# fanzyflani/pwnfps

Measured on AMD Instinct MI355X. Metric: Mpixels/s at 3840x2160 (level.txt scene, trace + blur), frames resident on the device; mean steps/ray alongside; d2h_inclusive = the rate with every frame delivered to the host (SURVEY 8d), higher is better.
Workload: dtype f32; 1 GPU; pwnfps level.txt scene (14 game.lua spheres, spawn pose, sec_current=0), 3840x2160, POSTPROC_BLUR=1, one frame per step; level=pwnfps_level, width=3840, height=2160, blur_passes=1, parallelism=rows/1, 3 frames in flight on two compute streams, frames_repeated_with_whole_strips=0

## Files before the change

include/pwnhip.h:

```cpp
#ifndef PWNHIP_H
#define PWNHIP_H
#include <stddef.h>
#include <stdint.h>

#ifdef __cplusplus
extern "C" {
#endif

#define PWN_OK            0
#define PWN_EINVAL       -1
#define PWN_ENODEV       -2
#define PWN_ENOMEM       -3
#define PWN_EIO          -4
#define PWN_EHIP         -5
#define PWN_ENOLEVEL     -6
#define PWN_ETOOBIG      -7
#define PWN_EBUSY        -8
#define PWN_ENOTSUP      -9
#define PWN_ETIMEDOUT    -10

typedef struct pwn_ctx pwn_ctx;

typedef struct pwn_portal { int32_t x1, z1, x2, z2, rot12, c1, c2; } pwn_portal;

// ... 50 lines not shown
	uint64_t frames, frames_redone, recuts;
	char note[160];
} pwn_group_info;
int pwn_init_multi(pwn_ctx **out, const int *devices, int ndev, int width, int height);
int pwn_group_info_get(pwn_ctx *ctx, pwn_group_info *out);
int pwn_set_option(pwn_ctx *ctx, int option, int value);
int pwn_unit_order_state(pwn_ctx *ctx, unsigned long long out[4]);
int pwn_unit_order_probe(pwn_ctx *ctx, const uint16_t *cost, uint32_t units, uint32_t *perm_out);
int pwn_launch_order_waits(pwn_ctx *ctx, unsigned long long *out);
int pwn_trace_room_state(pwn_ctx *ctx, int out[4]);
const char *pwn_strerror(int code);
const char *pwn_last_error(pwn_ctx *ctx);

int pwn_level_load(pwn_ctx *ctx, const char *path);
int pwn_level_load_mem(pwn_ctx *ctx, const char *text, int len);
int pwn_upload_level(pwn_ctx *ctx, const uint8_t data[4096], const pwn_portal pmap[26]);
int pwn_get_level(pwn_ctx *ctx, uint8_t data[4096], pwn_portal pmap[26], int32_t spawn[2]);

int pwn_upload_spheres(pwn_ctx *ctx, const pwn_sphere *spheres, int n);
int pwn_get_bins(pwn_ctx *ctx, uint16_t counts[4096], int32_t *idx, int cap);
#define PWN_TABLES_MAX (16u << 20)
#define PWN_LIST_MAX 4096
int pwn_sphere_tables_plan(const pwn_sphere *spheres, int n, unsigned long long out[6]);
int pwn_sphere_tables_state(pwn_ctx *ctx, unsigned long long out[6]);

#define PWN_OBJ_MAX 10000
int pwn_obj_new(pwn_ctx *ctx);
int pwn_obj_set_sphere(pwn_ctx *ctx, int obj, double r, double refl, double x, double y, double z,
	double cb, double cg, double cr);
int pwn_obj_free(pwn_ctx *ctx, int obj);
int pwn_level_get(pwn_ctx *ctx, int cx, int cz);
int pwn_prepare_render(pwn_ctx *ctx);
int pwn_get_objects(pwn_ctx *ctx, pwn_sphere *out, int cap);

int pwn_trace_screen_centred(pwn_ctx *ctx, const float cam[16], float sec_current,
	uint32_t *sbuf, float *zbuf);
int pwn_host_register(pwn_ctx *ctx, void *base, size_t bytes);
int pwn_host_unregister(pwn_ctx *ctx, void *base);
int pwn_call_strips_state(pwn_ctx *ctx, unsigned long long out[6]);

#define PWN_VIEWS_MAX 1024
int pwn_trace_views(pwn_ctx *ctx, int n, const float *cams, const float *secs, uint32_t *sbuf, float *zbuf);
#define PWN_VIEWS_HAS_W 1
int pwn_trace_views_device(pwn_ctx *ctx, int n, const void *d_cams, const void *d_secs, int flags,
	void *d_work, void *d_sbuf, void *d_zbuf, void *stream);

// ... 140 lines not shown
```

pwnfps_amd/__init__.py:

```python
from .render import (Renderer, PwnError, SPHERE_DTYPE, PORTAL_DTYPE, HIT_DTYPE,
                     mat4_iden, mat4_roty, mat4_rotx, spawn_camera, pixel_rays, unit_order_xy, sphere_tables_plan,
                     viewports_plan)
```

pwnfps_amd/_lib.py:

```python
import ctypes as C
import os

_HERE = os.path.dirname(os.path.abspath(__file__))
LIB_PATH = os.environ.get("PWNHIP_LIB") or os.path.join(_HERE, "libpwnhip.so")

PWN_OK, PWN_EINVAL, PWN_ENODEV, PWN_ENOMEM, PWN_EIO, PWN_EHIP, PWN_ENOLEVEL, PWN_ETOOBIG = 0, -1, -2, -3, -4, -5, -6, -7
PWN_EBUSY, PWN_ENOTSUP, PWN_ETIMEDOUT = -8, -9, -10
PWN_OPT_BLUR_PASSES, PWN_OPT_COUNTERS, PWN_OPT_SCHEDULER, PWN_OPT_REFILL_LIMIT, PWN_OPT_FRAME_TIMING, PWN_OPT_WAVE_LOG = 1, 2, 3, 4, 5, 6
PWN_OPT_FRAME_OVERLAP = 7
PWN_OPT_TRACE_ROOM = 8
PWN_OPT_UNIT_ORDER = 9
PWN_OPT_TILED_CHOREO = 10
PWN_OPT_TILED_STREAMS = 11
PWN_OPT_TILED_COMMS = 12
PWN_OPT_CALL_STRIPS = 13
PWN_TILED_CHOREO_INSTREAM, PWN_TILED_CHOREO_SPLIT = 0, 1
PWN_SCHED_UNITS, PWN_SCHED_REFILL = 0, 1
PWN_MAX_SLOTS = 4
PWN_FRAME_SBUF, PWN_FRAME_ZBUF, PWN_FRAME_SURFACE = 1, 2, 4
PWN_OBJ_MAX = 10000
PWN_TABLES_MAX = 16 << 20
PWN_VIEWS_MAX = 1024
PWN_RAYS_HAS_W = 1
PWN_VIEWS_HAS_W = 1
# ... 59 lines not shown
PWN_TILED_ID_BYTES = 128
PWN_TRANSPORT_RCCL, PWN_TRANSPORT_SHM, PWN_TRANSPORT_LOCAL = 0, 1, 2
PWN_TILED_HOST = 1
PWN_TILED_SLOTS = 6
PWN_TILED_MAX_WORLD = 64

_vp, _i, _f, _d = C.c_void_p, C.c_int, C.c_float, C.c_double
ABI = [
    ("pwn_init", _i, [C.POINTER(_vp), _i, _i, _i]),
    ("pwn_init_multi", _i, [C.POINTER(_vp), _vp, _i, _i, _i]),
    ("pwn_group_info_get", _i, [_vp, C.POINTER(GroupInfo)]),
    ("pwn_destroy", None, [_vp]),
    ("pwn_set_option", _i, [_vp, _i, _i]),
    ("pwn_trace_room_state", _i, [_vp, _vp]),
    ("pwn_strerror", C.c_char_p, [_i]),
    ("pwn_last_error", C.c_char_p, [_vp]),
    ("pwn_level_load", _i, [_vp, C.c_char_p]),
    ("pwn_level_load_mem", _i, [_vp, C.c_char_p, _i]),
    ("pwn_upload_level", _i, [_vp, _vp, _vp]),
    ("pwn_get_level", _i, [_vp, _vp, _vp, _vp]),
    ("pwn_upload_spheres", _i, [_vp, _vp, _i]),
    ("pwn_get_bins", _i, [_vp, _vp, _vp, _i]),
    ("pwn_sphere_tables_plan", _i, [_vp, _i, _vp]),
    ("pwn_sphere_tables_state", _i, [_vp, _vp]),
    ("pwn_obj_new", _i, [_vp]),
    ("pwn_obj_set_sphere", _i, [_vp, _i, _d, _d, _d, _d, _d, _d, _d, _d]),
    ("pwn_obj_free", _i, [_vp, _i]),
    ("pwn_level_get", _i, [_vp, _i, _i]),
    ("pwn_prepare_render", _i, [_vp]),
    ("pwn_get_objects", _i, [_vp, _vp, _i]),
    ("pwn_trace_screen_centred", _i, [_vp, _vp, _f, _vp, _vp]),
    ("pwn_host_register", _i, [_vp, _vp, C.c_size_t]),
    ("pwn_host_unregister", _i, [_vp, _vp]),
    ("pwn_call_strips_state", _i, [_vp, _vp]),
    ("pwn_trace_views", _i, [_vp, _i, _vp, _vp, _vp, _vp]),
    ("pwn_trace_views_device", _i, [_vp, _i, _vp, _vp, _i, _vp, _vp, _vp, _vp]),
    ("pwn_viewports_plan", _i, [_i, _i, _i, _i, _vp, _vp]),
    ("pwn_trace_viewports", _i, [_vp, _i, _vp, _vp, _vp, _vp, _vp]),
    ("pwn_pixel_rays", _i, [_i, _i, _vp, _i, _vp, _vp, _vp]),
    ("pwn_trace_rays", _i, [_vp, _i, _vp, _vp, _f, _vp, _vp]),
    ("pwn_trace_rays_device", _i, [_vp, _i, _vp, _vp, _f, _i, _vp, _vp, _vp]),
    ("pwn_trace_hits", _i, [_vp, _i, _vp, _vp]),
    ("pwn_trace_hits_device", _i, [_vp, _i, _vp, _i, _vp, _vp]),
    ("pwn_get_object_ids", _i, [_vp, _vp, _i]),
    ("pwn_frames_config", _i, [_vp, _i, _i, _i, _i]),
    ("pwn_submit_frame", _i, [_vp, _vp, _f, _i]),
# ... 51 lines not shown
```

pwnfps_amd/csrc/level_host.c:

```c
#include <stdint.h>
#include <stdlib.h>
#include <string.h>
#include "level_host.h"

enum { DIR_XP = 0, DIR_ZP, DIR_XN, DIR_ZN };

static int is_open(int c)
{
	switch(c)
	{
		case ';': case '$': case '"': case '#': case '&':
		case '>': case '<': case '^': case ',':
			return 1;
	}
	return 0;
}

static int flat_cell(const uint8_t *cells, int x, int z)
{
	int i = z * 64 + x;
	return (i >= 0 && i < 4096) ? cells[i] : '.';
}

static const int dir_dx[4] = { 1, 0, -1, 0 };
static const int dir_dz[4] = { 0, 1, 0, -1 };
// ... 156 lines not shown
			int x2 = trunc_to_int(s[i].x + s[i].r), z2 = trunc_to_int(s[i].z + s[i].r);
			if(x1 < 0) x1 = 0;
			if(z1 < 0) z1 = 0;
			if(x2 > 63) x2 = 63;
			if(z2 > 63) z2 = 63;
			for(int z = z1; z <= z2; z++)
			for(int x = x1; x <= x2; x++)
			{
				int c = z * 64 + x;
				if(pass == 0) off[c + 1]++;
				else idx[off[c] + fill[c]++] = i;
			}
		}
		if(pass == 0)
		{
			for(int c = 0; c < 4096; c++) off[c + 1] += off[c];
			if(idx == NULL) { free(fill); return off[4096]; }
			if(off[4096] > idx_cap) { free(fill); return -1; }
		}
	}
	free(fill);
	return off[4096];
}
```

pwnfps_amd/csrc/level_host.h:

```cpp
#ifndef PWN_LEVEL_HOST_H
#define PWN_LEVEL_HOST_H
#include <stdint.h>
#include "pwnhip.h"
#include "cell_bake.h"
#ifdef __cplusplus
extern "C" {
#endif
void pwn_level_clear(uint8_t *cells, pwn_portal *pmap, int32_t *spawn);
int pwn_parse_level(const char *text, int len, uint8_t *cells, pwn_portal *pmap, int32_t *spawn);
int pwn_check_portals(const uint8_t *cells, const pwn_portal *pmap);
int pwn_bake_cells(const uint8_t *cells, const pwn_portal *pmap, uint16_t *bits, uint32_t *recs);
int pwn_bin_spheres(const pwn_sphere *s, int n, int32_t *off, int32_t *idx, int idx_cap);
#ifdef __cplusplus
}
#endif
#endif
```

pwnfps_amd/csrc/pwn_api.cpp:

```cpp
#include <hip/hip_runtime.h>
#include <stdint.h>
#include <stdio.h>
#include <stdlib.h>
#include <string.h>
#include <time.h>
#include <new>
#include <algorithm>
#include <vector>
#include <xmmintrin.h>

#include "pwnhip.h"
#include "pwn_internal.h"
#include "level_host.h"
#include "approx_tables.inc"

extern "C" const char *pwn_strerror(int code)
{
	switch(code)
	{
		case PWN_OK: return "ok";
		case PWN_EINVAL: return "invalid argument";
		case PWN_ENODEV: return "no usable HIP device";
		case PWN_ENOMEM: return "out of memory";
		case PWN_EIO: return "level file could not be read";
// ... 23 lines not shown

#define GRP_HEAD(c) ((c) != NULL && (c)->grp != NULL && (c)->grp_head)
#define GRP_M0(c) pwn_group_member((c), 0)
#define GRP_REFUSE(c, what) do { if(GRP_HEAD(c)) { snprintf((c)->err, sizeof((c)->err), "%s is not available on a group's handle", what); return PWN_ENOTSUP; } } while(0)

extern "C" int pwn_init(pwn_ctx **out, int device, int width, int height)
{
	if(out == NULL || width <= 0 || height <= 0 || width > 32768 || height > 32768) return PWN_EINVAL;
	*out = NULL;
	int ndev = 0;
	if(hipGetDeviceCount(&ndev) != hipSuccess || ndev <= 0 || device < 0 || device >= ndev) return PWN_ENODEV;
	pwn_ctx *c = new(std::nothrow) pwn_ctx();
	if(c == NULL) return PWN_ENOMEM;
	c->device = device; c->w = width; c->h = height;
	c->blur_passes = 1; c->counters_on = 0; c->scheduler = PWN_SCHED_DEFAULT; c->refill_limit = PWN_REFILL_LIMIT_DEFAULT; c->have_level = false; c->cell_base_ok = false;
	if(const char *e = getenv("PWN_SCHEDULER")) c->scheduler = (strcmp(e, "refill") == 0 || strcmp(e, "1") == 0) ? PWN_SCHED_REFILL : PWN_SCHED_UNITS;
	if(const char *e = getenv("PWN_REFILL_LIMIT")) { int v = atoi(e); if(v >= 1 && v <= 64000) c->refill_limit = v; }
	c->dbg_force_hasw = getenv("PWN_DBG_FORCE_HASW") != NULL;
	c->dbg_blocks_per_cu = 0;
	c->dbg_blur_th = 0;
	if(const char *e = getenv("PWN_DBG_BLUR_TH")) c->dbg_blur_th = atoi(e);
	c->dbg_sphere_lists = 0; c->off_recsph = 0;
	c->dbg_sphere_lists = pwn_i_forced_lists();
	c->lists_form = PWN_LF_INDEXED; c->big_which = c->big_sph = 0; c->big_high = 0;
	for(int i = 0; i < PWN_NBLOB; i++) { c->d_big[i] = NULL; c->d_big_cap[i] = 0; }
	for(int i = 0; i < PWN_NSTAGE; i++) { c->h_big[i] = NULL; c->h_big_cap[i] = 0; }
	c->dbg_blur_tw = 0; c->dbg_blur_batch = -1;
	if(const char *e = getenv("PWN_DBG_BLUR_TW")) c->dbg_blur_tw = atoi(e);
	if(const char *e = getenv("PWN_DBG_BLUR_BATCH")) if(*e) c->dbg_blur_batch = atoi(e);
	if(const char *e = getenv("PWN_DBG_BLOCKS_PER_CU")) { int v = atoi(e); if(v > 0) c->dbg_blocks_per_cu = v; }
	c->blob_cur = 0; c->blob_dirty = true; c->off_sph = 0; c->stage_next = 0; c->up_stream = NULL;
	for(int i = 0; i < PWN_NBLOB; i++)
	{
		c->d_blob[i] = NULL; c->blob_has_static[i] = false;
		c->ev_tables[i] = NULL; c->tables_in_use[i] = false; c->tables_wait[i] = NULL;
		c->ev_upload[i] = NULL; c->upload_pending[i] = false;
	}
	for(int i = 0; i < PWN_NSTAGE; i++) { c->h_stage[i] = NULL; c->ev_stage[i] = NULL; c->stage_used[i] = false; }
	c->d_pre = c->d_out = NULL; c->d_z = NULL; c->d_skip = NULL; c->d_counters = NULL; c->d_tickets = NULL; c->ticket_set = 0; c->launch_rot = 2; c->launch_waits = 0;
	c->grid_reserve = 0;
	c->d_vpre = c->d_vout = NULL; c->d_vz = NULL; c->views_cap = 0; c->h_vrec = c->d_vrec = NULL; c->vrec_cap = 0; c->d_vrec_dev = NULL;
	c->d_ppre = c->d_pout = NULL; c->d_pz = NULL; c->h_prec = c->d_prec = NULL;
	c->h_rays = c->d_rays = NULL; c->rays_cap = 0;
	c->h_hits = c->d_hits = NULL; c->hits_cap = 0;
	memset(&c->room, 0, sizeof(c->room)); c->room.mode = -1;
	if(const char *e = getenv("PWN_TRACE_ROOM")) if(*e) c->room.mode = atoi(e) < 0 ? -1 : atoi(e);
// ... 372 lines not shown
			ci[(i >> 6) * PWN_GRID_PITCH + (i & 63)] |= PWN_C_SPH | (ord << 16);
			start[ord++] = (uint32_t)k0;
			for(int32_t k = k0; k < k1; k++)
			{
				const pwn_sphere &q = c->spheres[(size_t)c->bin_idx[k]];
				float r2 = q.r * q.r;
				if(r2 < 1.17549435e-38f) r2 = 0.0f;
				rec[4 * (size_t)k + 0] = q.x; rec[4 * (size_t)k + 1] = q.y; rec[4 * (size_t)k + 2] = q.z;
				uint32_t wbits;
				memcpy(&wbits, &r2, 4);
				if(k == k1 - 1) wbits |= 0x80000000u;
				memcpy(&rec[4 * (size_t)k + 3], &wbits, 4);
				which[k] = (uint32_t)c->bin_idx[k];
			}
		}
	}
	memcpy(b + PWN_T_RCP, c->tabs, 4096);
	memcpy(b + PWN_T_RSQ, c->tabs + 2048, 4096);
	pwn_fill_faces((float *)(b + PWN_T_FACES));
	memcpy(b + PWN_T_EPREC, c->ep_recs, sizeof(c->ep_recs));
	c->off_sph = glb ? 0u : (inl ? pwn_t_sph_offset_inl(nrec) : pwn_t_sph_offset(nbin));
	c->off_recsph = inl ? pwn_t_recsph_offset(nrec) : 0u;
	c->lists_form = plan.form;
	{
		float *sp = glb ? (float *)(c->big.data() + c->big_sph) : (float *)(b + c->off_sph);
		for(uint32_t i = 0; i < nsph; i++, sp += 8)
		{
			const pwn_sphere &q = c->spheres[i];
			float r2 = q.r * q.r;
			if(r2 < 1.17549435e-38f) r2 = 0.0f;
			sp[0] = q.x; sp[1] = q.y; sp[2] = q.z; sp[3] = r2;
			sp[4] = q.refl; sp[5] = q.cb; sp[6] = q.cg; sp[7] = q.cr;
		}
	}

	const int nb = (c->blob_cur + 1) % PWN_NBLOB;
	const uint32_t from = c->blob_has_static[nb] ? PWN_T_CELLINFO : 0u;
	const unsigned st = c->stage_next++ % PWN_NSTAGE;
	if(c->stage_used[st]) HIPCHK(c, hipEventSynchronize(c->ev_stage[st]));
	memcpy(c->h_stage[st], b + from, total - from);
	if(glb)
	{
		const int rc = big_reserve(c, nb, st, c->big.size());
		if(rc != PWN_OK) return rc;
		memcpy(c->h_big[st], c->big.data(), c->big.size());
	}
// ... 249 lines not shown
		if(n > cap) return PWN_EINVAL;
		for(int i = 0; i < n; i++) idx[i] = c->bin_idx[i];
	}
	return n;
}

static void plan_out(const pwn_tables_plan &p, unsigned long long out[6])
{
	out[0] = (unsigned long long)p.form;
	out[1] = (unsigned long long)p.blob_bytes + pwn_trace_lds_extra();
	out[2] = p.big_bytes;
	out[3] = p.nrec; out[4] = p.ncell; out[5] = p.longest;
}

extern "C" int pwn_sphere_tables_plan(const pwn_sphere *s, int n, unsigned long long out[6])
{
	if(out == NULL || n < 0 || n > PWN_OBJ_MAX || s == NULL) return PWN_EINVAL;
	std::vector<int32_t> off(4097, 0);
	if(pwn_bin_spheres(s, n, off.data(), NULL, 0) < 0) return PWN_ENOMEM;
	pwn_tables_plan p;
	const int rc = pwn_i_tables_plan(off.data(), (uint32_t)n, PWN_SCHED_DEFAULT, pwn_i_forced_lists(), &p);
	plan_out(p, out);
	return rc;
}

extern "C" int pwn_sphere_tables_state(pwn_ctx *c, unsigned long long out[6])
{
	if(GRP_HEAD(c)) { const int rc = pwn_group_sync(c); return rc != PWN_OK ? rc : pwn_sphere_tables_state(GRP_M0(c), out); }
	if(c == NULL || out == NULL) return PWN_EINVAL;
	pwn_tables_plan p;
	const int rc = pwn_i_tables_plan(c->bin_off.data(), (uint32_t)c->spheres.size(), c->scheduler, c->dbg_sphere_lists, &p);
	plan_out(p, out);
	return rc;
}



static void unit_div_magic(uint32_t d, uint32_t *magic, int *shift)
{
	*magic = 0u; *shift = -1;
	if(d < 2u) return;
	int s = 0;
	while((2u << s) < d) s++;
	const unsigned long long two = 1ull << (32 + s);
	const unsigned long long M = (two + d - 1u) / d;
	*magic = (uint32_t)M; *shift = s;
// ... 113 lines not shown
	{
		P.vps = vps->d_recs; P.nvp = vps->n; P.tiles_total = (int)vps->units;
		P.vp_step0 = 0u;
		if(vps->n > 1) { P.vp_step0 = 1u; while(2u * P.vp_step0 <= (uint32_t)vps->n - 1u) P.vp_step0 *= 2u; }
	}
	if(rays != NULL)
	{
		P.rays = rays->d_rays; P.ray_seeds = rays->d_seeds; P.nrays = rays->n; P.ray_w = rays->has_w ? 1 : 0;
		P.hits = rays->d_hits;
		P.tiles_total = (int)((rays->n + 63u) / 64u);
	}
	P.blob_bytes = (uint32_t)c->blob.size();
	P.off_sph = c->off_sph;
	P.off_recsph = c->off_recsph;
	P.sbuf = L->d_sbuf; P.zbuf = L->d_zbuf;
	const int cur = c->blob_cur;
	P.blob = (const uint32_t *)c->d_blob[cur];
	const bool glb = c->lists_form == PWN_LF_GLOBAL;
	if(glb)
	{
		P.g_rec = (const float *)c->d_big[cur];
		P.g_which = (const uint32_t *)(c->d_big[cur] + c->big_which);
		P.g_sph = (const float *)(c->d_big[cur] + c->big_sph);
	}
	if(c->upload_pending[cur])
	{
		if(hipEventQuery(c->ev_upload[cur]) == hipSuccess) c->upload_pending[cur] = false;
		else HIPCHK(c, hipStreamWaitEvent(stream, c->ev_upload[cur], 0));
	}
	P.counters = c->d_counters;
	P.clear_word = L->clear_word;
	P.cost_word = L->cost_word;
	P.wave_log = NULL;
	const unsigned rot = (unsigned)c->launch_rot, nsets = 2u * rot;
	P.tickets = c->d_tickets + (c->ticket_set % nsets) * PWN_QUEUES * PWN_QUEUE_STRIDE;
	P.tickets_next = c->d_tickets + ((c->ticket_set + rot) % nsets) * PWN_QUEUES * PWN_QUEUE_STRIDE;
	if(views != NULL) P.has_w = views->has_w;
	else if(rays != NULL) P.has_w = rays->has_w;
	else if(vps != NULL) P.has_w = vps->has_w;
	else P.has_w = !(L->cam[3] == 0.0f && L->cam[7] == 0.0f && L->cam[11] == 0.0f && L->cam[15] == 1.0f);
	if(c->dbg_force_hasw) P.has_w = 1;
	if(c->counters_on) HIPCHK(c, hipMemsetAsync(c->d_counters, 0, PWN_NCOUNTERS * sizeof(unsigned long long), stream));
	const bool refill = c->scheduler == PWN_SCHED_REFILL && !batch && !glb;
	const size_t lds_bytes = ((P.blob_bytes + 15u) & ~15u) + (refill ? pwn_trace_refill_lds_extra(P.has_w != 0) : pwn_trace_lds_extra());
	P.scheduler = c->scheduler;
	P.refill_limit = c->refill_limit;
// ... 1165 lines not shown
```

pwnfps_amd/csrc/pwn_internal.h:

```cpp
#pragma once
#include <hip/hip_runtime.h>
#include <stdint.h>
#include <stdio.h>
#include <vector>
#include <atomic>

#include "pwnhip.h"
#include "tables.h"

struct pwn_views_launch
{
	const pwn_view_rec *d_recs;
	int n;
	bool has_w;
	unsigned long long plane;
};

struct pwn_vps_launch
{
	const pwn_viewport_rec *d_recs, *h_recs;
	int n;
	bool has_w;
	uint32_t units;
};
// ... 125 lines not shown
	uint8_t cells[4096];
	uint32_t cell_base[65 * 65];
	bool cell_base_ok;
	uint32_t ep_recs[PWN_EP_MAX];
	pwn_portal pmap[26];
	int32_t spawn[2];
	std::vector<pwn_sphere> spheres;
	std::vector<int32_t> bin_off, bin_idx;
	std::vector<pwn_sphere> objs;
	std::vector<uint8_t> obj_typ;

	std::vector<uint8_t> blob;
	uint8_t *d_blob[PWN_NBLOB]; int blob_cur;
	bool blob_has_static[PWN_NBLOB];
	hipEvent_t ev_tables[PWN_NBLOB]; bool tables_in_use[PWN_NBLOB];
	hipEvent_t tables_wait[PWN_NBLOB];
	hipEvent_t ev_upload[PWN_NBLOB]; bool upload_pending[PWN_NBLOB];
	uint8_t *h_stage[PWN_NSTAGE]; hipEvent_t ev_stage[PWN_NSTAGE]; bool stage_used[PWN_NSTAGE]; unsigned stage_next;
	hipStream_t up_stream;
	uint16_t tabs[4096];
	uint32_t off_sph;
	uint32_t off_recsph; int dbg_sphere_lists;
	int lists_form;
	std::vector<uint8_t> big; uint64_t big_which, big_sph;
	uint8_t *d_big[PWN_NBLOB]; size_t d_big_cap[PWN_NBLOB];
	uint8_t *h_big[PWN_NSTAGE]; size_t h_big_cap[PWN_NSTAGE];
	size_t big_high;
	bool blob_dirty;
	size_t occ_lds[12]; int occ_blocks[12];

	uint32_t *d_pre, *d_out;
	float *d_z;
	uint2 *d_skip;
	unsigned long long *d_counters;
	unsigned long long *d_wave_log; int wave_log_on; size_t wave_log_cap;
	struct unit_order_state
	{
		hipStream_t key; bool used; unsigned long long stamp;
		uint16_t *d_cost; uint32_t *d_perm; size_t cost_cap, perm_cap;
		uint32_t units, qcap; int y0, y1;
		bool cost_fresh;
		uint32_t perm_units; int perm_y0, perm_y1; bool perm_valid;
	} order[4];
	unsigned long long order_stamp;
	int tiled_choreo;
	int tiled_streams;
// ... 101 lines not shown
```

pwnfps_amd/csrc/tables.h:

```cpp
#pragma once
#include <stdint.h>
#include "cell_bake.h"

#define PWN_GRID_PITCH 65u
#define PWN_T_RCP      0u
#define PWN_T_RSQ      4096u
#define PWN_T_FACES    8192u
#define PWN_T_EXP2     8448u
#define PWN_T_CELLINFO 8704u
#define PWN_T_EPREC    25616u
#define PWN_T_BINIDX   25824u

#define PWN_RCP_BASE   0x7e800000u
#define PWN_RSQ_BASE   0x5f000000u

#define PWN_C_ROOM   0x0100u
#define PWN_C_ROOM2  0x0200u
#define PWN_C_FOG    0x0400u
#define PWN_C_DQ     0x0800u
#define PWN_C_RAMP   0x1000u
#define PWN_C_RAMPX  0x2000u
#define PWN_C_RAMPM  0x4000u
#define PWN_C_PORTAL 0x8000u
#define PWN_C_SPH    0x80000000u
#define PWN_LIST_END 0xffffu
// ... 82 lines not shown
	int refill_limit;
	uint32_t *tickets, *tickets_next;
	uint32_t *cost_word;
	uint16_t *unit_cost;
	const uint32_t *perm;
	uint32_t perm_cap;
	uint32_t *clear_word;
	uint32_t off_recsph;
	const struct pwn_view_rec *views;
	int nviews;
	uint32_t views_magic; int views_shift;
	unsigned long long plane;
	const float *rays;
	const uint32_t *ray_seeds;
	uint32_t nrays;
	int ray_w;
	void *hits;
	const float *g_rec;
	const uint32_t *g_which;
	const float *g_sph;
	const struct pwn_viewport_rec *vps;
	int nvp;
	uint32_t vp_step0;
};
#define PWN_HIT_REC_BYTES 48u

struct pwn_blur_params
{
	int w, h, y0, y1;
	int groups;
	const uint32_t *pre;
	const float *zbuf;
	uint32_t *out;
	const uint2 *skip;
	int avail_y0, avail_y1;
	uint32_t *miss;
	int tile_h, tile_w, batch;
	uint32_t *cost_acc, *cost_out;
	uint32_t cost_mul, cost_div;
	int views;
	unsigned long long plane;
	const struct pwn_viewport_rec *vps;
	int nvp, vp_tiles;
};

enum { PWN_KM_FRAME = 0, PWN_KM_VIEWS = 1, PWN_KM_RAYS = 2, PWN_KM_HITS = 3, PWN_KM_VIEWPORTS = 4 };
// ... 27 lines not shown
```

pwnfps_amd/csrc/trace_common.h:

```cpp
#pragma once
#include <hip/hip_runtime.h>
#include <mutex>
#include "dev_math.h"
#include "tables.h"

#define EPS 0.0000000000001f
#define REFLECT_BLUR_F 0.03f
#define REFLECT_MAX 2
enum { FXP = 0, FZP, FXN, FZN, FYP, FYN };

#ifndef PWN_BLOCK
#define PWN_BLOCK 256
#endif
#define TILE_W 16
#define TILE_H 4

#ifndef PWN_MIN_WAVES
#define PWN_MIN_WAVES 3
#endif

#define PWN_LDS __attribute__((address_space(3)))
template<class T> __device__ __forceinline__ const PWN_LDS T *lds_at(uint32_t byte) { return (const PWN_LDS T *)(uintptr_t)byte; }
typedef float pwn_f4 __attribute__((ext_vector_type(4)));
struct Lds
{
	const PWN_LDS uint32_t *cellinfo;
	const PWN_LDS uint16_t *rcp, *rsq;
	const PWN_LDS unsigned char *eprec;
	const PWN_LDS uint16_t *binidx;
	const PWN_LDS uint16_t *recsph;
	const PWN_LDS float *sph;
	const PWN_LDS uint64_t *exp2;
	const PWN_LDS pwn_f4 *faces;
	const pwn_f4 *g_rec;
	const uint32_t *g_which;
	const pwn_f4 *g_sph;
};
__device__ __forceinline__ Lds lds_tables(uint32_t off_sph, uint32_t off_recsph = 0u)
{
	Lds L;
	L.cellinfo = lds_at<uint32_t>(PWN_T_CELLINFO);
	L.rcp = lds_at<uint16_t>(PWN_T_RCP);
	L.rsq = lds_at<uint16_t>(PWN_T_RSQ);
	L.eprec = lds_at<unsigned char>(PWN_T_EPREC - PWN_PST_REC0 * 4u);
// ... 69 lines not shown
	return r;
}
template<bool W> __device__ __forceinline__ Vec<W> vsub(const Vec<W> &a, const Vec<W> &b)
{
	Vec<W> r; r.x = a.x - b.x; r.y = a.y - b.y; r.z = a.z - b.z;
	if constexpr(W) r.w = a.w - b.w; else r.w = 0.0f;
	return r;
}
template<bool W> __device__ __forceinline__ Vec<W> vnormalise(const PWN_LDS uint16_t *rsq, const Vec<W> &a)
{
	return vscale<W>(tab_rsqrt(rsq, dot3<W>(a, a)), a);
}

__device__ __forceinline__ float dpp_row_shr1(float v)
{
	return __int_as_float(__builtin_amdgcn_update_dpp(0, __float_as_int(v), 0x111 , 0xf, 0xf, true));
}

enum { EV_NONE = 0, EV_WALL, EV_SPHERE, EV_EXHAUSTED };
enum { BASE_CEIL = 0, BASE_FLOOR, BASE_WALL, BASE_MAGENTA, BASE_ROOM_Y };

enum { RG_SEG = 0, RG_SETUP_SLOW, RG_EXHAUSTED, RG_WALL, RG_SPHERE, RG_FLOOR, RG_SPHREFL, RG_JITTER, RG_COMP1, RG_COMP1_FOG,
	RG_COMP2, RG_COMP2_FOG, RG_HELP, RG_UNIT, RG_SPHTEST, RG_SPHUPD, RG_ELSE,
	RG_UNIT_HALF, RG_HC_R2, RG_HC_OUT, RG_PORTAL_WALL, RG_PORTAL_GO, RG_PORTAL_ODD, RG_PORTAL_ROT2, RG_N };
struct Counters { uint32_t rays, steps, portals, tests, exhausted, wsteps, wp[8], apasses, apass_lanes, rg[RG_N]; };
#define WAVE_PATH(k) do { if(COUNT && (__ffsll((long long)__ballot(1)) - 1) == (int)(threadIdx.x & 63)) cnt.wp[k]++; } while(0)
#define RG(k) do { if(COUNT && (__ffsll((long long)__ballot(1)) - 1) == (int)(threadIdx.x & 63)) cnt.rg[k]++; } while(0)


__device__ __forceinline__ uint32_t pixel_seed(int x, int y, int w)
{
	uint32_t seed = (uint32_t)x + (uint32_t)y * (uint32_t)y * ((uint32_t)w + 1u);
	seed *= seed * seed;
	seed *= seed * seed;
	return seed << 1;
}

__device__ __forceinline__ void blob_to_lds(unsigned char *lds, const void *blob, uint32_t blob_bytes)
{
	const uint4 *src = (const uint4 *)blob;
	uint4 *dst = (uint4 *)lds;
	int n16 = (int)(blob_bytes >> 4);
	for(int i = threadIdx.x; i < n16; i += PWN_BLOCK) dst[i] = src[i];
}

__device__ __forceinline__ uint32_t next_open_queue(uint32_t q, unsigned long long open)
{
// ... 75 lines not shown
```

pwnfps_amd/csrc/trace_walk.inc:

```
#define AUX_HIT() (cdist > aux_dist)
if(COUNT)
{
	cnt.steps++;
	if((__ffsll((long long)__ballot(1)) - 1) == (int)(threadIdx.x & 63)) cnt.wsteps++;
}

if constexpr(HITREC) hit_cxz = cxz;

#ifdef PWN_PLAIN_STATS
if(COUNT)
{
	const bool sp1 = ((int)cw < 0) || !(cw & PWN_C_ROOM);
	const bool sp2 = sp1 || (cw & (PWN_C_ROOM2 | PWN_C_DQ)) != 0u;
	const bool low = (__ffsll((long long)__ballot(1)) - 1) == (int)(threadIdx.x & 63);
	if(__ballot(sp1) == 0ull && low) cnt.apasses++;
	if(__ballot(sp2) == 0ull && low) cnt.apass_lanes++;
}
#endif

if((int)cw < 0)
{
	WAVE_PATH(0);
	if constexpr(LISTS == PWN_LF_GLOBAL)
	{
		uint32_t ri = ((const PWN_LDS uint32_t *)L.binidx)[(cw >> 16) & 0x7fffu];
		pwn_f4 nx = L.g_rec[(size_t)ri];
		for(;;)
		{
			RG(RG_SPHTEST);
			const pwn_f4 s0 = nx;
			const uint32_t wb = __float_as_uint(s0.w);
			nx = L.g_rec[(size_t)ri + 1u];
#define PWN_ST_RAD2 __uint_as_float(wb & 0x7fffffffu)
#define PWN_ST_WHICH ri
#include "trace_sphere.inc"
#undef PWN_ST_RAD2
#undef PWN_ST_WHICH
			if((int)wb < 0) break;
			ri++;
		}
	}
	else if constexpr(LISTS == PWN_LF_INLINE)
	{
		const PWN_LDS pwn_f4 *rp = (const PWN_LDS pwn_f4 *)L.binidx + ((cw >> 16) & 0x7fffu);
		pwn_f4 nx = *rp;
		for(;;)
// ... 228 lines not shown
```

pwnfps_amd/render.py:

```python
import ctypes as C

import numpy as np

from . import _lib
from ._lib import lib

HIT_DTYPE = np.dtype([("kind", "<i4"), ("face", "<i4"), ("object", "<i4"), ("portals", "<i4"),
                      ("dist", "<f4"), ("x", "<f4"), ("y", "<f4"), ("z", "<f4"),
                      ("dx", "<f4"), ("dy", "<f4"), ("dz", "<f4"), ("cell_x", "<i2"), ("cell_z", "<i2")])
SPHERE_DTYPE = np.dtype([("r", "<f4"), ("refl", "<f4"), ("x", "<f4"), ("y", "<f4"),
                         ("z", "<f4"), ("cb", "<f4"), ("cg", "<f4"), ("cr", "<f4")])
PORTAL_DTYPE = np.dtype([(n, "<i4") for n in ("x1", "z1", "x2", "z2", "rot12", "c1", "c2")])


class PwnError(RuntimeError):
    def __init__(self, code, where, detail=""):
        self.code = code
        msg = "%s: %s (%d)" % (where, lib.pwn_strerror(code).decode(), code)
        if detail:
            msg += ": " + detail
        super().__init__(msg)


class Renderer:
# ... 514 lines not shown
        words = np.ascontiguousarray(words).view(np.uint32).ravel()
        per = {_lib.PROBE_DIV: 2, _lib.PROBE_FTOINT: 4}.get(op, 1)
        n = words.size // per
        out = np.zeros(n, np.uint32)
        self._chk(lib.pwn_probe(self._ctx, int(op), words.ctypes.data, out.ctypes.data, n), "pwn_probe")
        return out


def _tables_dict(out):
    return {"form": int(out[0]), "lds_bytes": int(out[1]), "device_bytes": int(out[2]), "pairs": int(out[3]),
            "cells": int(out[4]), "longest": int(out[5])}


def sphere_tables_plan(spheres):
    spheres = np.ascontiguousarray(spheres, SPHERE_DTYPE)
    out = (C.c_uint64 * 6)()
    buf = spheres if len(spheres) else np.zeros(1, SPHERE_DTYPE)
    rc = lib.pwn_sphere_tables_plan(buf.ctypes.data, len(spheres), out)
    if rc < 0:
        raise PwnError(rc, "pwn_sphere_tables_plan")
    return _tables_dict(out)


def _rect_records(rects, who):
    rects = np.asarray(rects)
    if rects.ndim != 2 or rects.shape[1] != 4 or rects.shape[0] < 1:
        raise ValueError("%s: rects must have shape (n,4) with n >= 1, not %s" % (who, rects.shape))
    if rects.shape[0] > _lib.PWN_VIEWS_MAX:
        raise ValueError("%s: %d rectangles, at most %d" % (who, rects.shape[0], _lib.PWN_VIEWS_MAX))
    return np.ascontiguousarray(rects, np.int32)


def viewports_plan(W, H, rects, blur):
    rects = _rect_records(rects, "viewports_plan")
    out = (C.c_uint64 * 4)()
    rc = lib.pwn_viewports_plan(int(W), int(H), int(blur), rects.shape[0], rects.ctypes.data, out)
    if rc not in (_lib.PWN_OK, _lib.PWN_EINVAL):
        raise PwnError(rc, "pwn_viewports_plan")
    return {"ok": rc == _lib.PWN_OK, "units": int(out[0]), "pixels": int(out[1]), "largest": int(out[2]), "offender": int(out[3])}


def _ray_records(rays, who):
    if isinstance(rays, (tuple, list)) and len(rays) == 2:
        o, d = np.asarray(rays[0]), np.asarray(rays[1])
        if o.ndim != 2 or d.ndim != 2 or o.shape[0] != d.shape[0] or o.shape[1] not in (3, 4) or d.shape[1] not in (3, 4):
            raise ValueError("%s: origins and directions must be (n,3) or (n,4) with the same n, not %s and %s" % (who, o.shape, d.shape))
# ... 94 lines not shown
```

Measured before the change: 26610 Mpixels/s.

## Cull dense sphere cells with wave-uniform bounding-sphere test

On the host, builds up to four bounding spheres around the most populated sphere-list cells and passes them through the kernel arguments. In the trace walk, when a whole wavefront shares a cell list with such a bound, it runs one conservative ray-vs-bound test. If no lane can hit the bound, it skips the per-sphere tests for that cell. This adds a kernarg read, a ballot and a branch per sphere cell, and relies on the bound staying conservative for correctness.

```diff
diff --git a/include/pwnhip.h b/include/pwnhip.h
--- a/include/pwnhip.h
+++ b/include/pwnhip.h
@@ -96,6 +96,8 @@
 #define PWN_TABLES_MAX (16u << 20)
 #define PWN_LIST_MAX 4096
 int pwn_sphere_tables_plan(const pwn_sphere *spheres, int n, unsigned long long out[6]);
+#define PWN_BOUNDS_MAX 4
+int pwn_sphere_bounds_plan(const pwn_sphere *spheres, int n, double out[PWN_BOUNDS_MAX][8]);
 int pwn_sphere_tables_state(pwn_ctx *ctx, unsigned long long out[6]);
 
 #define PWN_OBJ_MAX 10000
diff --git a/pwnfps_amd/__init__.py b/pwnfps_amd/__init__.py
--- a/pwnfps_amd/__init__.py
+++ b/pwnfps_amd/__init__.py
@@ -1,3 +1,3 @@
 from .render import (Renderer, PwnError, SPHERE_DTYPE, PORTAL_DTYPE, HIT_DTYPE,
-                     mat4_iden, mat4_roty, mat4_rotx, spawn_camera, pixel_rays, unit_order_xy, sphere_tables_plan,
+                     mat4_iden, mat4_roty, mat4_rotx, spawn_camera, pixel_rays, unit_order_xy, sphere_tables_plan, sphere_bounds_plan,
                      viewports_plan)
diff --git a/pwnfps_amd/_lib.py b/pwnfps_amd/_lib.py
--- a/pwnfps_amd/_lib.py
+++ b/pwnfps_amd/_lib.py
@@ -105,6 +105,7 @@
     ("pwn_upload_spheres", _i, [_vp, _vp, _i]),
     ("pwn_get_bins", _i, [_vp, _vp, _vp, _i]),
     ("pwn_sphere_tables_plan", _i, [_vp, _i, _vp]),
+    ("pwn_sphere_bounds_plan", _i, [_vp, _i, _vp]),
     ("pwn_sphere_tables_state", _i, [_vp, _vp]),
     ("pwn_obj_new", _i, [_vp]),
     ("pwn_obj_set_sphere", _i, [_vp, _i, _d, _d, _d, _d, _d, _d, _d, _d]),
diff --git a/pwnfps_amd/csrc/level_host.c b/pwnfps_amd/csrc/level_host.c
--- a/pwnfps_amd/csrc/level_host.c
+++ b/pwnfps_amd/csrc/level_host.c
@@ -1,6 +1,7 @@
 #include <stdint.h>
 #include <stdlib.h>
 #include <string.h>
+#include <math.h>
 #include "level_host.h"
 
 enum { DIR_XP = 0, DIR_ZP, DIR_XN, DIR_ZN };
@@ -203,3 +204,61 @@
 	free(fill);
 	return off[4096];
 }
+
+int pwn_sphere_bounds_build(const pwn_sphere *s, const int32_t *off, const int32_t *idx, int form, pwn_sphere_bound *out)
+{
+	int pick[PWN_BOUNDS_MAX], npick = 0;
+	for(int k = 0; k < PWN_BOUNDS_MAX; k++)
+	{
+		int best = -1, best_n = PWN_BOUND_MIN_RECORDS - 1;
+		for(int c = 0; c < 4096; c++)
+		{
+			const int n = off[c + 1] - off[c];
+			if(n <= best_n) continue;
+			int taken = 0;
+			for(int j = 0; j < npick; j++) taken |= pick[j] == c;
+			if(!taken) { best = c; best_n = n; }
+		}
+		if(best < 0) break;
+		pick[npick++] = best;
+	}
+	int nout = 0;
+	for(int k = 0; k < npick; k++)
+	{
+		const int cell = pick[k], k0 = off[cell], k1 = off[cell + 1], n = k1 - k0;
+		uint32_t id = 0;
+		for(int c = 0; c < cell; c++)
+		{
+			const int m = off[c + 1] - off[c];
+			if(m > 0) id += form == 0 ? (uint32_t)m + 1u : (form == 1 ? (uint32_t)m : 1u);
+		}
+		int ok = 1;
+		double mx = 0.0, my = 0.0, mz = 0.0;
+		for(int i = k0; i < k1; i++)
+		{
+			const pwn_sphere *q = &s[idx[i]];
+			const double v[4] = { q->x, q->y, q->z, q->r };
+			for(int j = 0; j < 4; j++) if(!(fabs(v[j]) <= PWN_SB_COORD_LIMIT)) ok = 0;
+			mx += q->x; my += q->y; mz += q->z;
+		}
+		if(!ok) continue;
+		const float cx = (float)(mx / n), cy = (float)(my / n), cz = (float)(mz / n);
+		double reff = 0.0;
+		for(int i = k0; i < k1; i++)
+		{
+			const pwn_sphere *q = &s[idx[i]];
+			const double dx = (double)q->x - cx, dy = (double)q->y - cy, dz = (double)q->z - cz;
+			const double rho = sqrt(dx * dx + dy * dy + dz * dz) * (1.0 + 1e-12), r = fabs((double)q->r);
+			if(!(rho + r <= PWN_SB_R_LIMIT)) ok = 0;
+			const double a = PWN_SB_D_MAX + rho;
+			const double r0 = rho + sqrt(r * r + PWN_SB_EPS_PROOF * a * a + PWN_SB_ETA);
+			if(r0 > reff) reff = r0;
+		}
+		if(!ok) continue;
+		const float rf = nextafterf((float)(reff * (1.0 + 1.0 / 1048576.0)), INFINITY);
+		const float rr = nextafterf((float)((double)rf * (double)rf), INFINITY);
+		pwn_sphere_bound *b = &out[nout++];
+		b->id = id; b->count = (uint32_t)n; b->cx = cx; b->cy = cy; b->cz = cz; b->rr = rr; b->neg_r = -rf; b->cell = (uint32_t)cell;
+	}
+	return nout;
+}
diff --git a/pwnfps_amd/csrc/level_host.h b/pwnfps_amd/csrc/level_host.h
--- a/pwnfps_amd/csrc/level_host.h
+++ b/pwnfps_amd/csrc/level_host.h
@@ -3,6 +3,7 @@
 #include <stdint.h>
 #include "pwnhip.h"
 #include "cell_bake.h"
+#include "sphere_bound.h"
 #ifdef __cplusplus
 extern "C" {
 #endif
@@ -11,6 +12,7 @@
 int pwn_check_portals(const uint8_t *cells, const pwn_portal *pmap);
 int pwn_bake_cells(const uint8_t *cells, const pwn_portal *pmap, uint16_t *bits, uint32_t *recs);
 int pwn_bin_spheres(const pwn_sphere *s, int n, int32_t *off, int32_t *idx, int idx_cap);
+int pwn_sphere_bounds_build(const pwn_sphere *s, const int32_t *off, const int32_t *idx, int form, pwn_sphere_bound *out);
 #ifdef __cplusplus
 }
 #endif
diff --git a/pwnfps_amd/csrc/pwn_api.cpp b/pwnfps_amd/csrc/pwn_api.cpp
--- a/pwnfps_amd/csrc/pwn_api.cpp
+++ b/pwnfps_amd/csrc/pwn_api.cpp
@@ -69,6 +69,8 @@
 	if(const char *e = getenv("PWN_DBG_BLUR_TH")) c->dbg_blur_th = atoi(e);
 	c->dbg_sphere_lists = 0; c->off_recsph = 0;
 	c->dbg_sphere_lists = pwn_i_forced_lists();
+	c->nbounds = 0;
+	{ const char *e = getenv("PWN_SPHERE_BOUNDS"); c->dbg_sphere_bounds = (e != NULL && strcmp(e, "0") == 0) ? 0 : 1; }
 	c->lists_form = PWN_LF_INDEXED; c->big_which = c->big_sph = 0; c->big_high = 0;
 	for(int i = 0; i < PWN_NBLOB; i++) { c->d_big[i] = NULL; c->d_big_cap[i] = 0; }
 	for(int i = 0; i < PWN_NSTAGE; i++) { c->h_big[i] = NULL; c->h_big_cap[i] = 0; }
@@ -487,6 +489,8 @@
 	c->off_sph = glb ? 0u : (inl ? pwn_t_sph_offset_inl(nrec) : pwn_t_sph_offset(nbin));
 	c->off_recsph = inl ? pwn_t_recsph_offset(nrec) : 0u;
 	c->lists_form = plan.form;
+	static_assert(PWN_LF_INDEXED == 0 && PWN_LF_INLINE == 1 && PWN_LF_GLOBAL == 2, "pwn_sphere_bounds_build takes the form as a number");
+	c->nbounds = nsph > 0u ? pwn_sphere_bounds_build(c->spheres.data(), c->bin_off.data(), c->bin_idx.data(), plan.form, c->bounds) : 0;
 	{
 		float *sp = glb ? (float *)(c->big.data() + c->big_sph) : (float *)(b + c->off_sph);
 		for(uint32_t i = 0; i < nsph; i++, sp += 8)
@@ -782,6 +786,29 @@
 	const int rc = pwn_i_tables_plan(off.data(), (uint32_t)n, PWN_SCHED_DEFAULT, pwn_i_forced_lists(), &p);
 	plan_out(p, out);
 	return rc;
+}
+
+extern "C" int pwn_sphere_bounds_plan(const pwn_sphere *s, int n, double out[PWN_BOUNDS_MAX][8])
+{
+	if(out == NULL || n < 0 || n > PWN_OBJ_MAX || s == NULL) return PWN_EINVAL;
+	std::vector<int32_t> off(4097, 0);
+	const int nb = pwn_bin_spheres(s, n, off.data(), NULL, 0);
+	if(nb < 0) return PWN_ENOMEM;
+	pwn_tables_plan p;
+	const int rc = pwn_i_tables_plan(off.data(), (uint32_t)n, PWN_SCHED_DEFAULT, pwn_i_forced_lists(), &p);
+	if(rc != PWN_OK) return rc;
+	std::vector<int32_t> idx((size_t)(nb > 0 ? nb : 1));
+	if(pwn_bin_spheres(s, n, off.data(), idx.data(), nb) != nb) return PWN_ENOMEM;
+	pwn_sphere_bound b[PWN_BOUNDS_MAX];
+	const int k = n > 0 ? pwn_sphere_bounds_build(s, off.data(), idx.data(), p.form, b) : 0;
+	memset(out, 0, sizeof(double) * PWN_BOUNDS_MAX * 8);
+	for(int i = 0; i < k; i++)
+	{
+		double *o = out[i];
+		o[0] = (double)b[i].cell; o[1] = (double)b[i].count; o[2] = (double)b[i].id;
+		o[3] = b[i].cx; o[4] = b[i].cy; o[5] = b[i].cz; o[6] = -(double)b[i].neg_r; o[7] = b[i].rr;
+	}
+	return k;
 }
 
 extern "C" int pwn_sphere_tables_state(pwn_ctx *c, unsigned long long out[6])
@@ -941,6 +968,12 @@
 		P.g_rec = (const float *)c->d_big[cur];
 		P.g_which = (const uint32_t *)(c->d_big[cur] + c->big_which);
 		P.g_sph = (const float *)(c->d_big[cur] + c->big_sph);
+	}
+	P.nbounds = c->dbg_sphere_bounds ? c->nbounds : 0;
+	for(int i = 0; i < PWN_BOUNDS_MAX; i++)
+	{
+		P.bound_ids[i] = 0xffffffffu;
+		if(i < P.nbounds) { P.bounds[i] = c->bounds[i]; P.bound_ids[i] = c->bounds[i].id; }
 	}
 	if(c->upload_pending[cur])
 	{
diff --git a/pwnfps_amd/csrc/pwn_internal.h b/pwnfps_amd/csrc/pwn_internal.h
--- a/pwnfps_amd/csrc/pwn_internal.h
+++ b/pwnfps_amd/csrc/pwn_internal.h
@@ -171,6 +171,8 @@
 	uint32_t off_sph;
 	uint32_t off_recsph; int dbg_sphere_lists;
 	int lists_form;
+	pwn_sphere_bound bounds[PWN_BOUNDS_MAX]; int nbounds;
+	int dbg_sphere_bounds;
 	std::vector<uint8_t> big; uint64_t big_which, big_sph;
 	uint8_t *d_big[PWN_NBLOB]; size_t d_big_cap[PWN_NBLOB];
 	uint8_t *h_big[PWN_NSTAGE]; size_t h_big_cap[PWN_NSTAGE];
diff --git a/pwnfps_amd/csrc/sphere_bound.h b/pwnfps_amd/csrc/sphere_bound.h
--- /dev/null
+++ b/pwnfps_amd/csrc/sphere_bound.h
@@ -0,0 +1,57 @@
+#ifndef PWN_SPHERE_BOUND_H
+#define PWN_SPHERE_BOUND_H
+#include <stdint.h>
+
+#ifndef PWN_BOUNDS_MAX
+#define PWN_BOUNDS_MAX 4
+#endif
+#define PWN_BOUND_MIN_RECORDS 4
+#define PWN_SB_RAY_EPS    0.0009765625f
+#define PWN_SB_D2_MAX     4.0f
+#define PWN_SB_EPS_PROOF  1.0e-3
+#define PWN_SB_ETA        0.000244140625
+#define PWN_SB_D_MAX      2.001
+#define PWN_SB_R_LIMIT    1.5
+#define PWN_SB_COORD_LIMIT 1024.0
+
+typedef struct pwn_sphere_bound
+{
+	uint32_t id;
+	uint32_t count;
+	float cx, cy, cz;
+	float rr;
+	float neg_r;
+	uint32_t cell;
+} pwn_sphere_bound;
+
+#ifdef __HIPCC__
+#define PWN_SB_FN __device__ __host__ __forceinline__
+#else
+#define PWN_SB_FN static inline
+#endif
+
+PWN_SB_FN int pwn_sb_pass(int has_w, float px, float py, float pz, float pw, float rx, float ry, float rz, float rw,
+	float cx, float cy, float cz, float rr, float neg_r)
+{
+	const float ex = cx - px, ey = cy - py, ez = cz - pz;
+	float d2c, dtc, l2;
+	if(has_w)
+	{
+		const float ew = 1.0f - pw;
+		d2c = (ex * ex + ez * ez) + (ey * ey + ew * ew);
+		dtc = (ex * rx + ez * rz) + (ey * ry + ew * rw);
+		l2 = (rx * rx + rz * rz) + (ry * ry + rw * rw);
+	}
+	else
+	{
+		d2c = (ex * ex + ez * ez) + ey * ey;
+		dtc = (ex * rx + ez * rz) + ey * ry;
+		l2 = (rx * rx + rz * rz) + ry * ry;
+	}
+	const float dl = l2 - 1.0f;
+	const int g1 = d2c <= PWN_SB_D2_MAX;
+	const int g2 = (dl <= PWN_SB_RAY_EPS) & (dl >= -PWN_SB_RAY_EPS);
+	const int miss = (dtc <= neg_r) | (d2c - dtc * dtc >= rr);
+	return !(g1 & g2 & miss);
+}
+#endif
diff --git a/pwnfps_amd/csrc/tables.h b/pwnfps_amd/csrc/tables.h
--- a/pwnfps_amd/csrc/tables.h
+++ b/pwnfps_amd/csrc/tables.h
@@ -1,6 +1,7 @@
 #pragma once
 #include <stdint.h>
 #include "cell_bake.h"
+#include "sphere_bound.h"
 
 #define PWN_GRID_PITCH 65u
 #define PWN_T_RCP      0u
@@ -129,6 +130,9 @@
 	const struct pwn_viewport_rec *vps;
 	int nvp;
 	uint32_t vp_step0;
+	int nbounds;
+	uint32_t bound_ids[PWN_BOUNDS_MAX];
+	pwn_sphere_bound bounds[PWN_BOUNDS_MAX];
 };
 #define PWN_HIT_REC_BYTES 48u
 
diff --git a/pwnfps_amd/csrc/trace_common.h b/pwnfps_amd/csrc/trace_common.h
--- a/pwnfps_amd/csrc/trace_common.h
+++ b/pwnfps_amd/csrc/trace_common.h
@@ -20,6 +20,7 @@
 #endif
 
 #define PWN_LDS __attribute__((address_space(3)))
+#define PWN_KARGS __attribute__((address_space(4)))
 template<class T> __device__ __forceinline__ const PWN_LDS T *lds_at(uint32_t byte) { return (const PWN_LDS T *)(uintptr_t)byte; }
 typedef float pwn_f4 __attribute__((ext_vector_type(4)));
 struct Lds
@@ -135,7 +136,9 @@
 
 enum { RG_SEG = 0, RG_SETUP_SLOW, RG_EXHAUSTED, RG_WALL, RG_SPHERE, RG_FLOOR, RG_SPHREFL, RG_JITTER, RG_COMP1, RG_COMP1_FOG,
 	RG_COMP2, RG_COMP2_FOG, RG_HELP, RG_UNIT, RG_SPHTEST, RG_SPHUPD, RG_ELSE,
-	RG_UNIT_HALF, RG_HC_R2, RG_HC_OUT, RG_PORTAL_WALL, RG_PORTAL_GO, RG_PORTAL_ODD, RG_PORTAL_ROT2, RG_N };
+	RG_UNIT_HALF, RG_HC_R2, RG_HC_OUT, RG_PORTAL_WALL, RG_PORTAL_GO, RG_PORTAL_ODD, RG_PORTAL_ROT2,
+	RG_SPHBOUND, RG_SPHSKIP,
+	RG_N };
 struct Counters { uint32_t rays, steps, portals, tests, exhausted, wsteps, wp[8], apasses, apass_lanes, rg[RG_N]; };
 #define WAVE_PATH(k) do { if(COUNT && (__ffsll((long long)__ballot(1)) - 1) == (int)(threadIdx.x & 63)) cnt.wp[k]++; } while(0)
 #define RG(k) do { if(COUNT && (__ffsll((long long)__ballot(1)) - 1) == (int)(threadIdx.x & 63)) cnt.rg[k]++; } while(0)
diff --git a/pwnfps_amd/csrc/trace_walk.inc b/pwnfps_amd/csrc/trace_walk.inc
--- a/pwnfps_amd/csrc/trace_walk.inc
+++ b/pwnfps_amd/csrc/trace_walk.inc
@@ -21,7 +21,35 @@
 if((int)cw < 0)
 {
 	WAVE_PATH(0);
-	if constexpr(LISTS == PWN_LF_GLOBAL)
+	bool sb_skip = false;
+	{
+		const PWN_KARGS pwn_trace_params *KP = (const PWN_KARGS pwn_trace_params *)__builtin_amdgcn_kernarg_segment_ptr();
+		if(KP->nbounds != 0)
+		{
+			const uint32_t lid = (cw >> 16) & 0x7fffu;
+			const uint32_t id0 = (uint32_t)__builtin_amdgcn_readfirstlane((int)lid);
+			if(__ballot(lid != id0) == 0ull)
+			{
+				int k = -1;
+#pragma unroll
+				for(int i = PWN_BOUNDS_MAX - 1; i >= 0; i--) if(KP->bound_ids[i] == id0) k = i;
+				if(k >= 0)
+				{
+					RG(RG_SPHBOUND);
+					const PWN_KARGS pwn_sphere_bound *sb = &KP->bounds[k];
+					const int pass = pwn_sb_pass(HAS_W, pos.x, pos.y, pos.z, pos.w, ray.x, ray.y, ray.z, ray.w, sb->cx, sb->cy, sb->cz, sb->rr, sb->neg_r);
+					if(__ballot(pass) == 0ull)
+					{
+						RG(RG_SPHSKIP);
+						sb_skip = true;
+						if(COUNT) cnt.tests += sb->count;
+					}
+				}
+			}
+		}
+	}
+	if(sb_skip) { }
+	else if constexpr(LISTS == PWN_LF_GLOBAL)
 	{
 		uint32_t ri = ((const PWN_LDS uint32_t *)L.binidx)[(cw >> 16) & 0x7fffu];
 		pwn_f4 nx = L.g_rec[(size_t)ri];
diff --git a/pwnfps_amd/render.py b/pwnfps_amd/render.py
--- a/pwnfps_amd/render.py
+++ b/pwnfps_amd/render.py
@@ -560,6 +560,17 @@
     return _tables_dict(out)
 
 
+def sphere_bounds_plan(spheres):
+    spheres = np.ascontiguousarray(spheres, SPHERE_DTYPE)
+    out = np.zeros((4, 8), np.float64)
+    buf = spheres if len(spheres) else np.zeros(1, SPHERE_DTYPE)
+    rc = lib.pwn_sphere_bounds_plan(buf.ctypes.data, len(spheres), out.ctypes.data)
+    if rc < 0:
+        raise PwnError(rc, "pwn_sphere_bounds_plan")
+    return [{"cell": int(o[0]), "records": int(o[1]), "id": int(o[2]), "centre": (float(o[3]), float(o[4]), float(o[5])),
+             "r_eff": float(o[6]), "rr": float(o[7])} for o in out[:rc]]
+
+
 def _rect_records(rects, who):
     rects = np.asarray(rects)
     if rects.ndim != 2 or rects.shape[1] != 4 or rects.shape[0] < 1:
```

Measured after the change: 28090 Mpixels/s (median of 6 runs). +5.6%, better.
